# DRSY/EasyKV

Measured on AMD Instinct MI355X. Metric: decode_tokens_per_sec, higher is better.
Workload: dtype f16 storage / f32 accumulate; 1 GPU; bench-D decode at fixed budget: B=1 L=32 Hq=32 H=32 D=128 budget=2048 T=2049 kv_policy=roco (Llama2-7B shape, budget=50% of S=4096); parallelism=1 GPU, layers_per_launch=32, layers_per_rank=32, sequences_per_launch=1, n_split=1, fused=True, slot_map=scattered (random permutation: long-run steady state), prewarm_steps=4096, hipgraph=False, overlap_scorer=False, handoff=False

## Files before the change

easykv_amd/_lib.py:

```python
from __future__ import annotations

import ctypes as C
import os

import torch

from ._build import LIB

POLICY_NONE, POLICY_H2O_HEAD, POLICY_ROCO, POLICY_TOVA, POLICY_RANGE = 0, 1, 2, 3, 4
PHASE_SLOT_TAIL_OK = 32
PHASE_SLOT_ROWS = 16
POLICY_CODES = {"full": POLICY_NONE, "h2o_head": POLICY_H2O_HEAD, "roco": POLICY_ROCO, "tova": POLICY_TOVA,
                "recency": POLICY_RANGE, "random": POLICY_RANGE}

DTYPE_F16, DTYPE_BF16 = 0, 1
DTYPE_CODES = {torch.float16: DTYPE_F16, torch.bfloat16: DTYPE_BF16}

MAX_SEQS = 64
DTYPE_F32 = 2
STEP_CALLS = ("step_check", "step_info", "workspace_bytes", "step_attend")


def step_call_name(rows, batch, what):
    if rows is None and not batch:
        return "ekv_" + what + "_typed"
    return "ekv_" + (rows + "_" if rows else "") + ("batch_" if batch else "") + what


EXPORTS = ("ekv_abi_version", "ekv_strerror", "ekv_workspace_bytes", "ekv_step_plan", "ekv_bank_reset", "ekv_state_init",
           "ekv_step_attend", "ekv_gather_ordered", "ekv_scatter_rows", "ekv_compact_inplace", "ekv_step_check", "ekv_step_info",
           "ekv_rows_to_slots", "ekv_rows_to_order", "ekv_kv8_quantize", "ekv_kv8_dequantize", "ekv_kv4_quantize", "ekv_kv4_dequantize",
           "ekv_kv6_quantize", "ekv_kv6_dequantize", "ekv_set_resident_bytes", "ekv_step_resident_rows", "ekv_kv84_quantize", "ekv_kv84_dequantize",
           "ekv_kv164_quantize", "ekv_kv164_dequantize") + tuple(
               step_call_name(rows, batch, what) for rows in (None, "kv8", "kv4", "kv6", "kv84", "kv164") for batch in (False, True) for what in STEP_CALLS)
LONG_CALLS = {what: "ekv_long_" + what for what in STEP_CALLS}
EXPORTS += tuple(LONG_CALLS[what] for what in STEP_CALLS)
LONG_INFO_N = 12
CAP_CALLS = {what: "ekv_cap_" + what for what in STEP_CALLS}
EXPORTS += tuple(CAP_CALLS[what] for what in STEP_CALLS) + ("ekv_softcap_eval",)
SINK_CALLS = {what: "ekv_sink_" + what for what in STEP_CALLS}
EXPORTS += tuple(SINK_CALLS[what] for what in STEP_CALLS)
WIN_CALLS = {what: "ekv_win_" + what for what in STEP_CALLS}
EXPORTS += tuple(WIN_CALLS[what] for what in STEP_CALLS)
POOL_CALLS = {what: "ekv_pool_" + what for what in STEP_CALLS}
EXPORTS += tuple(POOL_CALLS[what] for what in STEP_CALLS)
POOL_OPS = {"max": 0, "avg": 1}

# ... 72 lines not shown
    lib.ekv_workspace_bytes.restype = C.c_size_t
    lib.ekv_workspace_bytes.argtypes = [C.POINTER(Bank), C.POINTER(Step)]
    lib.ekv_step_plan.argtypes = [C.POINTER(Bank), C.POINTER(Step), C.POINTER(C.c_int32), C.POINTER(C.c_int32)]
    lib.ekv_bank_reset.argtypes = [C.POINTER(Bank), vp]
    lib.ekv_state_init.argtypes = [C.POINTER(Bank), i32, i32, i32, i32, i32, vp]
    lib.ekv_step_attend.argtypes = [C.POINTER(Bank), C.POINTER(Step), vp, vp, vp, vp, vp, vp, vp, vp, C.c_size_t, vp]
    lib.ekv_gather_ordered.argtypes = [C.POINTER(Bank), i32, i32, i32, vp, vp, vp]
    lib.ekv_scatter_rows.argtypes = [C.POINTER(Bank), i32, i32, i32, i32, vp, vp, vp]
    lib.ekv_compact_inplace.argtypes = [C.POINTER(Bank), i32, i32, i32, i32, vp, vp]
    lib.ekv_step_check.argtypes = [C.POINTER(Bank), C.POINTER(Step)]
    lib.ekv_step_info.argtypes = [C.POINTER(Bank), C.POINTER(Step), C.POINTER(C.c_int32), C.c_int32]
    lib.ekv_rows_to_slots.argtypes = [C.POINTER(Bank), i32, i32, i32, vp]
    lib.ekv_rows_to_order.argtypes = [C.POINTER(Bank), i32, i32, i32, vp]
    lib.ekv_set_resident_bytes.argtypes = [C.c_int64]
    lib.ekv_step_resident_rows.argtypes = [C.POINTER(Bank), C.POINTER(Step), i32]
    tails = {"step_check": [], "workspace_bytes": [], "step_info": [C.POINTER(C.c_int32), C.c_int32]}
    for rows, desc in ((None, None), ("kv8", Kv8), ("kv4", Kv4), ("kv6", Kv6), ("kv84", Kv84), ("kv164", Kv164)):
        for batch in (False, True):
            head = [C.POINTER(Bank), C.POINTER(Step), i32] + ([C.POINTER(desc)] if desc else []) + ([C.POINTER(Seq), i32] if batch else [])
            tails["step_attend"] = [vp] * (6 if batch else 8) + [C.c_size_t, vp]
            for what in STEP_CALLS:
                getattr(lib, step_call_name(rows, batch, what)).argtypes = head + tails[what]
        if rows is None:
            tails["step_attend"] = [vp] * 8 + [C.c_size_t, vp]
            for what in STEP_CALLS:
                getattr(lib, LONG_CALLS[what]).argtypes = [C.POINTER(Bank), C.POINTER(Step), i32] + tails[what]
                getattr(lib, CAP_CALLS[what]).argtypes = [C.POINTER(Bank), C.POINTER(Step), i32, C.c_float] + tails[what]
                getattr(lib, SINK_CALLS[what]).argtypes = [C.POINTER(Bank), C.POINTER(Step), i32, vp] + tails[what]
                getattr(lib, WIN_CALLS[what]).argtypes = [C.POINTER(Bank), C.POINTER(Step), i32, C.POINTER(Win)] + tails[what]
                getattr(lib, POOL_CALLS[what]).argtypes = [C.POINTER(Bank), C.POINTER(Step), i32, C.POINTER(Pool)] + tails[what]
# ... 25 lines not shown
```

easykv_amd/csrc/ekv_abi.hip:

```cpp
#include "ekv_common.h"
#include "ekv_kernels.h"
#include "ekv_plan.h"

static inline void drop_stale_error() { (void)hipGetLastError(); }
static inline int launch_code(hipError_t e) { return e == hipSuccess ? EKV_OK : EKV_E_LAUNCH; }

static int call_attend(const EkvCall& c, const void* q, const void* k_new, const void* v_new, void* out, int32_t* evict_ids,
                       const float* rope_cos, const float* rope_sin, void* workspace, size_t workspace_bytes, void* stream) {
  EkvResolved r;
  if (int e = resolve_call(c, &r)) return e;
  const ekv_bank* bank = r.bank;
  const ekv_step* st = r.step;
  const EkvSeqTable* tb = r.tb;
  const EkvStepPlan& P = r.plan;
  if (!q || !k_new || !v_new || !out || !workspace || (st->rope_on_read && (!rope_cos || !rope_sin))) return EKV_E_ARG;
  if (P.bytes > workspace_bytes) return EKV_E_WORKSPACE;
  hipStream_t s = static_cast<hipStream_t>(stream);
  const int n = st->q_len, D = bank->head_dim, lc = st->layer_count;
  char* const ws = static_cast<char*>(workspace);
  auto f32 = [&](int64_t off) { return off < 0 ? nullptr : reinterpret_cast<float*>(ws + off); };
  auto f16 = [&](int64_t off) { return off < 0 ? nullptr : reinterpret_cast<__half*>(ws + off); };

  EkvAttnArgs aa{};
  aa.k = static_cast<const __half*>(bank->k);
// ... 65 lines not shown
  const float* const sinks = P.sink ? c.sinks : nullptr;
  const bool window = P.window != 0;
  const EkvWinArgs win = window ? EkvWinArgs{c.win->tok_pos, c.win->windows, c.win->q_pos0} : EkvWinArgs{};
  drop_stale_error();
  for (int i = 0; i < P.n_list; ++i) {
    const EkvLaunch& L = P.list[i];
    sa.skip_fold = L.skip_fold;
    hipError_t e = hipSuccess;
    if (window && (L.kind == EKV_RUN_CHUNK_LDS || L.kind == EKV_RUN_RESIDENT || L.kind == EKV_RUN_FLUSH || (L.kind == EKV_RUN_CHUNK && P.wide))) return EKV_E_UNSUPPORTED;
    if (rows != EKV_ROWS_kv16 && (L.kind == EKV_RUN_CHUNK_LDS || L.kind == EKV_RUN_RESIDENT || L.kind == EKV_RUN_CHUNK || L.kind == EKV_RUN_FLUSH)) return EKV_E_UNSUPPORTED;
    if (sinks && (L.kind == EKV_RUN_CHUNK_LDS || L.kind == EKV_RUN_RESIDENT || L.kind == EKV_RUN_FLUSH || (L.kind == EKV_RUN_CHUNK && P.wide))) return EKV_E_UNSUPPORTED;
    if (capped && (L.kind == EKV_RUN_CHUNK_LDS || L.kind == EKV_RUN_RESIDENT || L.kind == EKV_RUN_FLUSH || (L.kind == EKV_RUN_CHUNK && P.wide))) return EKV_E_UNSUPPORTED;
    switch (L.kind) {
      case EKV_RUN_FUSED_DECODE:
        aa.fused_order = P.fused_order;
        e = window ? ekv_launch_decode_fused_win(aa, sa, sinks, win, D, lc, P.fused_nw, s, bf16)
          : sinks ? ekv_launch_decode_fused_sink(aa, sa, sinks, D, lc, P.fused_nw, s, bf16)
                  : ekv_launch_decode_fused(aa, sa, tb, D, lc, P.fused_nw, s, bf16, rows, capped);
        break;
      case EKV_RUN_CHUNK_LDS: e = ekv_launch_chunk_lds(aa, sa, D, lc, s, bf16); break;
      case EKV_RUN_RESIDENT: e = ekv_launch_attn_resident(aa, sa, lc, s, bf16); break;
      case EKV_RUN_DECODE:
        e = window ? ekv_launch_attn_decode_win(aa, sinks, win, D, lc, s, bf16)
          : sinks ? ekv_launch_attn_decode_sink(aa, sinks, D, lc, s, bf16) : ekv_launch_attn_decode(aa, tb, D, lc, s, bf16, rows, capped);
        break;
      case EKV_RUN_CHUNK:
        e = window ? ekv_launch_attn_chunk_win(aa, sinks, win, D, lc, P.two_pass, s, L.fuse ? &sa : nullptr, bf16)
          : sinks ? ekv_launch_attn_chunk_sink(aa, sinks, D, lc, P.two_pass, s, L.fuse ? &sa : nullptr, bf16)
                  : ekv_launch_attn_chunk(aa, D, lc, P.wide, P.two_pass, s, L.fuse ? &sa : nullptr, L.passes, L.tail ? &sa : nullptr, bf16, capped);
        break;
// ... 37 lines not shown

int ekv_step_plan(const ekv_bank* bank, const ekv_step* st, int32_t* n_split, int32_t* fused) { return call_plan(bank, st, n_split, fused); }

int ekv_step_info_typed(const ekv_bank* bank, const ekv_step* st, int32_t dtype, int32_t* info, int32_t n_info) {
  return call_info(step_call(bank, st, dtype), info, n_info);
}
int ekv_step_info(const ekv_bank* bank, const ekv_step* st, int32_t* info, int32_t n_info) {
  return call_info(step_call(bank, st, EKV_DTYPE_F16), info, n_info);
}

int ekv_set_resident_bytes(int64_t bytes) {
  ekv_resident_set_budget_bytes(bytes);
  return EKV_OK;
}
int ekv_step_resident_rows(const ekv_bank* bank, const ekv_step* st, int32_t dtype) { return call_resident_rows(step_call(bank, st, dtype)); }

int ekv_step_check_typed(const ekv_bank* bank, const ekv_step* st, int32_t dtype) { return call_check(step_call(bank, st, dtype)); }
int ekv_step_check(const ekv_bank* bank, const ekv_step* st) { return call_check(step_call(bank, st, EKV_DTYPE_F16)); }

int ekv_step_attend(const ekv_bank* bank, const ekv_step* st, const void* q, const void* k_new, const void* v_new,
                    void* out, int32_t* evict_ids, const float* rope_cos, const float* rope_sin, void* workspace,
                    size_t workspace_bytes, void* stream) {
  return call_attend(step_call(bank, st, EKV_DTYPE_F16), q, k_new, v_new, out, evict_ids, rope_cos, rope_sin, workspace, workspace_bytes, stream);
}
int ekv_step_attend_typed(const ekv_bank* bank, const ekv_step* st, int32_t dtype, const void* q, const void* k_new,
                          const void* v_new, void* out, int32_t* evict_ids, const float* rope_cos, const float* rope_sin,
                          void* workspace, size_t workspace_bytes, void* stream) {
  return call_attend(step_call(bank, st, dtype), q, k_new, v_new, out, evict_ids, rope_cos, rope_sin, workspace, workspace_bytes, stream);
}

// ... 398 lines not shown
```

easykv_amd/csrc/ekv_attn_decode.inc:

```
#ifdef EKV_TAIL_PROFILE
#define EKV_STAMP(i) do { if (threadIdx.x == 0) stamps[i] = __builtin_readcyclecounter(); } while (0)
#endif
#include "ekv_decode_stream.h"
#include "ekv_decode_tail.h"
#ifndef EKV_KV8
#define EKV_KV8 0
#endif
#ifndef EKV_BATCH
#define EKV_BATCH 0
#endif
#ifndef EKV_KV4
#define EKV_KV4 0
#endif
#ifndef EKV_KV6
#define EKV_KV6 0
#endif
#if EKV_KV4 || EKV_KV6
#define EKV_MX 1
#else
#define EKV_MX 0
#endif
#ifndef EKV_KV84
#define EKV_KV84 0
#endif
// ... 125 lines not shown
  const int lane = tid & 63, wave = tid >> 6;
  const int T = a.n_slots;
  const int nrep = (REP == 1 || REP == 2) ? REP : a.n_q_heads / a.n_kv_heads;
  const bool roco = sc.policy == EKV_POLICY_ROCO;
  const bool scored = roco || sc.policy == EKV_POLICY_H2O_HEAD || sc.policy == EKV_POLICY_TOVA;
  const int off = scored ? sc.score_off : 0;
  const int W = SLOT ? a.phys_extent : T - off;
  const int w_pad = (int)ekv_align((size_t)W, 256);
#ifdef EKV_NO_PHYS
  constexpr bool PHYS = false;
#else
  constexpr bool PHYS = !ROPE;
#endif
  const int l_pad = a.l_pad;
  constexpr bool kResident = D == 128 && REP == 1 && PHYS && SLOT && !EKV_G8 && !EKV_MX && !EKV_KV164 && !EKV_BATCH && !EKV_SINK && !EKV_WINDOW;
  const int res_rows = kResident ? EKV_RESIDENT_ROWS(a.fused_order) : 0;
  float* s_logit = reinterpret_cast<float*>(smem);
  float* s_part = s_logit + (size_t)REP * l_pad;
  float* sS = s_part + (size_t)Gm::NP * REP * Gm::PS + ((Gm::NP * REP * Gm::PS) & 3 ? 4 - ((Gm::NP * REP * Gm::PS) & 3) : 0);
  float* sQ = sS + w_pad;
  float* sC = sQ + w_pad;
  RedN<NW> red;
  red.buf = reinterpret_cast<unsigned long long*>(sS + (size_t)(roco ? (SLOT ? 2 : 3) : 1) * w_pad);
  red.phase = 0;
  red.lane = lane;
  red.wave = wave;
  const size_t head_row = ((size_t)(a.layer_begin + ll) * a.n_kv_heads + h) * a.cap;
#ifdef EKV_TAIL_PROFILE
  unsigned long long* stamps = reinterpret_cast<unsigned long long*>(sc.tova_row) + ((size_t)ll * a.n_kv_heads + h) * 8;
#endif
  EKV_STAMP(0);
  constexpr bool kOrders = D == 128 && REP == 1 && !ROPE && ((NW == 4 && ITEMS <= 12) || (NW == 8 && !EKV_SOFTCAP && (ITEMS <= 5 || ITEMS == 13))) && SLOT && !EKV_G8 && !EKV_MX && !EKV_KV164 && !EKV_BATCH && !EKV_SINK && !EKV_WINDOW;
  bool order_k = false;
  if constexpr (kOrders) {
    const int om = a.fused_order & 3;
    if (om == 2) {
      order_k = scored;
    } else if (om == 1 && scored) {
      uint32_t* s_flag = reinterpret_cast<uint32_t*>(red.buf);
      if (tid == 0) {
        const uint32_t hw = __builtin_amdgcn_s_getreg(63492);
        const int src = (a.fused_order >> 4) & 3;
        const uint32_t x = src == 0 ? (hw >> 16) & 15u : (src == 1 ? hw & 15u : (uint32_t)(ll * a.n_kv_heads + h));
        bool below = (x & ((a.fused_order >> 8) & 15u)) < ((a.fused_order >> 12) & 15u);
        if constexpr (NW == 8)
          if (src == 3) below = x < (uint32_t)EKV_ORDER_ROUND_THRESHOLD(a.fused_order);
        *s_flag = below != (((a.fused_order >> 6) & 1) != 0) ? 1u : 0u;
      }
      __syncthreads();
      order_k = __builtin_amdgcn_readfirstlane((int)*s_flag) != 0;
    }
  }
// ... 45 lines not shown
      float mk = EKV_NEG_INF;
      ekv_decode_plane_loop<D, NW, kResident>(a.k, head_row, E, mask_ready, [&](uint4 (&kr)[8], const int j0) {
        const unsigned dead8 = (unsigned)s_dead[j0 >> 3];
        float s[8];
#pragma unroll
        for (int u = 0; u < 8; ++u) {
          const float acc = ekv_group_sum<LPR>(ekv_dot8(qv, kr[u], 0.f));
          s[u] = !((dead8 >> u) & 1u) ? EKV_LOGIT(acc, a) : EKV_NEG_INF;
        }
        float mine = s[0];
#pragma unroll
        for (int u = 1; u < 8; ++u) mine = (sub == u) ? s[u] : mine;
        if (sub < 8 && !((dead8 >> sub) & 1u)) s_logit[j0 + sub] = mine;
#pragma unroll
        for (int u = 0; u < 8; ++u) mk = fmaxf(mk, s[u]);
      }, res_rows);
      const __half* v_new_row = a.v_new + ((size_t)ll * a.n_kv_heads + h) * D;
      if (wave == 0 && grp == 0) {
        const uint4 kn = reinterpret_cast<const uint4*>(a.k_new + ((size_t)ll * a.n_kv_heads + h) * D)[sub];
        const uint4 vn = reinterpret_cast<const uint4*>(v_new_row)[sub];
        const size_t off_new = (head_row + new_row) * D;
        reinterpret_cast<uint4*>(a.k_w + off_new)[sub] = kn;
        reinterpret_cast<uint4*>(a.v_w + off_new)[sub] = vn;
        const float acc = EKV_LOGIT(ekv_group_sum<LPR>(ekv_dot8(qv, kn, 0.f)), a);
        if (sub == 0) s_logit[new_row] = acc;
        mk = fmaxf(mk, acc);
      }
      ekv_tail_prefetch_ragged<NW>(sc, head_row, W, roco, sS, sQ, sC, false);
      if constexpr (kLateHeadState) EKV_HEAD_STATE();
      float cC[ITEMS];
      int32_t cB[ITEMS];
// ... 37 lines not shown
#pragma unroll
        for (int u = 1; u < 8; ++u) mx = fmaxf(mx, s[u]);
        const float mn = fmaxf(m[0], mx);
        if (mn == EKV_NEG_INF) return;
        const float alpha = exp2f((m[0] - mn) * EKV_LOG2E);
        l[0] *= alpha;
#pragma unroll
        for (int i = 0; i < 8; ++i) o[0][i] *= alpha;
#pragma unroll
        for (int u = 0; u < 8; ++u) {
          const float p = exp2f((s[u] - mn) * EKV_LOG2E);
          l[0] += p;
          ekv_axpy8(p, vr[u], o[0]);
        }
        m[0] = mn;
      }, res_rows);
      if (wave == 0 && grp == 0) {
        const uint4 vn = reinterpret_cast<const uint4*>(v_new_row)[sub];
        const float acc = s_logit[new_row];
        const float mn = fmaxf(m[0], acc);
        const float alpha = m[0] == EKV_NEG_INF ? 0.f : exp2f((m[0] - mn) * EKV_LOG2E);
        const float p = exp2f((acc - mn) * EKV_LOG2E);
        l[0] = l[0] * alpha + p;
#pragma unroll
        for (int i = 0; i < 8; ++i) o[0][i] *= alpha;
        ekv_axpy8(p, vn, o[0]);
        m[0] = mn;
      }
      ekv_decode_wave_combine<D, 1>(m, l, o);
      ekv_decode_stash<D, 1, NW>(s_part, m, l, o);
      __syncthreads();
// ... 213 lines not shown
```

easykv_amd/csrc/ekv_decode_stream.h:

```cpp
#pragma once
#include "ekv_common.h"
#include "ekv_kernels.h"


struct EkvNoop {
  __device__ __forceinline__ void operator()() const {}
};
#ifndef EKV_ROPE_MOCK
#define EKV_ROPE_MOCK 0
#endif
template <bool RESIDENT>
__device__ __forceinline__ uint4 ekv_load_row_piece(const char* row, int sub) {
  const ekv_u4* p = reinterpret_cast<const ekv_u4*>(row) + sub;
  if constexpr (RESIDENT) return __builtin_bit_cast(uint4, *p);
  else return __builtin_bit_cast(uint4, __builtin_nontemporal_load(p));
}
template <bool B>
struct EkvBool {
  static constexpr bool value = B;
};

template <int D, int REP, bool ROPE, bool SLOT_LDS, int NW = 4, bool PHYS = false, int KU = kU, typename MaskReady = EkvNoop, int EPL = 8, int FMT = 0, bool RES = false>
__device__ __forceinline__ void ekv_decode_stream(const EkvAttnArgs& a, const int32_t* s_slot, float* logit_out,
                                                  int logit_stride, int t0, int t1_in, int ll, int h, size_t head_row,
// ... 546 lines not shown
  ls = 0.f;
  os = 0.f;
#pragma unroll
  for (int i = 0; i < Gm::NP; ++i) {
    const float* p = s_part + ((size_t)i * REP + r) * Gm::PS;
    const float w = (p[0] == EKV_NEG_INF) ? 0.f : exp2f((p[0] - mm) * EKV_LOG2E);
    ls += p[1] * w;
    os += p[2 + d] * w;
  }
}

template <int D, int NW, bool RES = false, typename First, typename Consume>
__device__ __forceinline__ void ekv_decode_plane_loop(const __half* plane, size_t head_row, int t1, First&& first, Consume&& consume, int res_rows = 0) {
  using Gm = EkvDecodeGeom<D, NW, 8, 8>;
  static_assert(Gm::LIVE == Gm::LPR, "whole lane groups");
  constexpr int RW = Gm::RW, STEP = NW * RW;
  const int lane = threadIdx.x & 63, wave = threadIdx.x >> 6;
  const int sub = lane % Gm::LPR, grp = lane / Gm::LPR;
  auto request_as = [&](auto resident, uint4 (&r)[8], int base) {
    int j0 = base + grp * 8;
    if constexpr (RES) asm volatile("" : "+v"(j0));
#pragma unroll
    for (int u = 0; u < 8; ++u) {
      const int row = j0 + u < t1 ? j0 + u : t1 - 1;
      const char* p = reinterpret_cast<const char*>(plane) + (head_row + row) * (D * 2);
      r[u] = ekv_load_row_piece<decltype(resident)::value>(p, sub);
    }
  };
  auto request = [&](uint4 (&r)[8], int base) {
    if constexpr (RES) {
      if (min(base, t1 - 1) < res_rows) request_as(EkvBool<true>(), r, base);
      else request_as(EkvBool<false>(), r, base);
    } else {
      request_as(EkvBool<false>(), r, base);
    }
  };
  uint4 ra[8], rb[8];
  int base = wave * RW;
  request(ra, base);
  first();
  while (base < t1) {
    request(rb, base + STEP);
    consume(ra, base + grp * 8);
    base += STEP;
    if (base >= t1) break;
    request(ra, base + STEP);
// ... 5 lines not shown
```

easykv_amd/csrc/ekv_kernels.h:

```cpp
#pragma once
#include <hip/hip_runtime.h>
#include <hip/hip_fp16.h>
#include <stdint.h>

#include "../../include/easykv_hip.h"
#include "ekv_geometry.h"

enum EkvRows : int32_t { EKV_ROWS_kv16, EKV_ROWS_kv8, EKV_ROWS_kv4, EKV_ROWS_kv6, EKV_ROWS_kv84, EKV_ROWS_kv164 };

#define EKV_RESIDENT_UNIT 32
#define EKV_RESIDENT_BITS(rows) ((((rows) / EKV_RESIDENT_UNIT) > 255 ? 255 : ((rows) / EKV_RESIDENT_UNIT)) << 16)
#define EKV_RESIDENT_ROWS(order) ((((order) >> 16) & 255) * EKV_RESIDENT_UNIT)
#define EKV_ORDER_ROUND_UNIT 8
#define EKV_ORDER_ROUND_BITS(wgs) \
  (((((wgs) / EKV_ORDER_ROUND_UNIT > 255 ? 255 : (wgs) / EKV_ORDER_ROUND_UNIT) >> 4) << 8) | ((((wgs) / EKV_ORDER_ROUND_UNIT > 255 ? 255 : (wgs) / EKV_ORDER_ROUND_UNIT) & 15) << 12))
#define EKV_ORDER_ROUND_THRESHOLD(order) ((((((order) >> 8) & 15) << 4) | (((order) >> 12) & 15)) * EKV_ORDER_ROUND_UNIT)

enum EkvLaunchKind : int32_t {
  EKV_RUN_FUSED_DECODE,
  EKV_RUN_CHUNK_LDS,
  EKV_RUN_RESIDENT,
  EKV_RUN_DECODE,
  EKV_RUN_CHUNK,
  EKV_RUN_FLUSH,
  EKV_RUN_FOLD, EKV_RUN_RANGE, EKV_RUN_DECODE_SCORE, EKV_RUN_TOVA_MEAN, EKV_RUN_SCORE_SELECT,
  EKV_RUN_LONG_FOLD,
  EKV_RUN_LONG_SCORE
// ... 29 lines not shown
  int64_t big_rows;
  int64_t stats, colsum, row_stats;
  int64_t q_keep;
  int64_t q_rot;
  size_t bytes;
  int32_t one_launch;
  int32_t n_launches;
  int32_t n_list;
  EkvLaunch list[6];
  int32_t long_rows, long_tiles;
  int64_t key_rows;
  int32_t capped;
  int32_t sink;
  int32_t window;
  int32_t pooled;
};
struct EkvSeqTable {
  ekv_seq e[EKV_MAX_SEQS];
};

struct EkvAttnArgs {
  const __half* k;
  const __half* v;
  __half* k_w;
  __half* v_w;
  const int32_t* slot_of_pos;
  const __half* q;
  const __half* k_new;
  const __half* v_new;
  float* logits;
// ... 17 lines not shown
  int32_t n_col_parts;
  int32_t n_q_heads, n_kv_heads, cap, n_slots, q_len, n_split, rows_per_split, t_pad, layer_begin, causal;
  int32_t qb_rows, n_qblocks;
  int32_t phys_extent;
  int32_t l_pad;
  uint32_t* arrive;
  float sm_div;
  float softcap;
  __half* q_keep;
  int32_t new_in_cache;
  union {
    int32_t score_tail;
    int32_t fused_order;
  };
  int32_t q_ts, q_hs, kv_ts, kv_hs, o_ts, o_hs;
  int32_t n_stat_parts;
};

struct EkvScoreArgs {
  int32_t* slot_of_pos;
  float* score_sum;
  float* score_sq;
  float* score_cnt;
  const float* logits;
  const float* partials;
  const float* colsum;
  float* big_rows;
  int big_stride;
  const float* row_stats;
  int32_t n_col_parts;
  float* tova_row;
// ... 213 lines not shown
```

easykv_amd/csrc/ekv_plan.cpp:

```cpp
#include "ekv_plan.h"

#include <algorithm>
#include <cstdio>
#include <cstdlib>

namespace {

typedef int64_t i64;

bool env_is_1(const char* name) { const char* e = std::getenv(name); return e != nullptr && e[0] == '1'; }
int env_int(const char* name, int otherwise) { const char* e = std::getenv(name); return e != nullptr ? std::atoi(e) : otherwise; }

bool pow2_to_16(int rep) { return rep == 1 || rep == 2 || rep == 4 || rep == 8 || rep == 16; }

}

int check_bank(const ekv_bank* b) {
  if (!b || !b->k || !b->v || !b->slot_of_pos) return EKV_E_ARG;
  if (b->n_layers <= 0 || b->n_kv_heads <= 0 || b->n_q_heads % b->n_kv_heads || b->cap <= 0) return EKV_E_ARG;
  if (b->head_dim != 32 && b->head_dim != 64 && b->head_dim != 96 && b->head_dim != 128 && b->head_dim != 256) return EKV_E_UNSUPPORTED;
  return EKV_OK;
}

int check_layers(const ekv_bank* b, int begin, int count) {
// ... 56 lines not shown
  return n_heads_in_launch >= 512 ? (1 | rule4) : 0;
}

#ifndef EKV_RESIDENT_MB_DEFAULT
#define EKV_RESIDENT_MB_DEFAULT 224
#endif
namespace {
i64 g_resident_bytes = -1;
}
i64 ekv_resident_budget_bytes() {
  static const i64 dflt = (i64)std::max(0, std::min(env_int("EKV_RESIDENT_MB", EKV_RESIDENT_MB_DEFAULT), 1 << 20)) << 20;
  return g_resident_bytes < 0 ? dflt : g_resident_bytes;
}
void ekv_resident_set_budget_bytes(i64 bytes) { g_resident_bytes = bytes; }

int ekv_decode_resident_rows(i64 n_heads_in_launch, i64 row_bytes, int phys_extent, int cap, int score_rows, i64 budget_bytes) {
  static const int force = env_int("EKV_RESIDENT_ROWS", -1);
  if (n_heads_in_launch <= 0 || row_bytes <= 0 || phys_extent <= 0 || cap <= 0 || score_rows < 0) return 0;
  const i64 unit = EKV_RESIDENT_UNIT;
  const i64 ext = std::min<i64>(((i64)phys_extent + unit - 1) / unit * unit, 255 * unit);
  if (budget_bytes <= 0) return 0;
  if (force >= 0) return (int)std::min<i64>(force / unit * unit, ext);
  const i64 heads = std::min<i64>(n_heads_in_launch, 1 << 20);
  const i64 score = heads * 4 * cap * (score_rows + 2);
  const i64 per_unit = heads * 2 * unit * std::min<i64>(row_bytes, 1 << 16);
  if (budget_bytes < score) return 0;
  return (int)(std::min<i64>((budget_bytes - score) / per_unit, ext / unit) * unit);
}

bool ekv_decode_fused_supported(int head_dim, int rep, int n_slots, int t_pad, int l_pad, int n_evict, int cap, int nw) {
  if (!ekv_attn_decode_supported(head_dim, rep) || rep > 8 || n_evict > 1 || n_slots > 256 * 24 || (cap & 3) != 0 || cap < 16) return false;
  size_t lds = 1 << 30;
  switch (head_dim) {
    case 32: lds = ekv_fused_lds_max<32>(rep, t_pad, l_pad, nw); break;
    case 64: lds = ekv_fused_lds_max<64>(rep, t_pad, l_pad, nw); break;
    case 96: lds = ekv_fused_lds_max<96>(rep, t_pad, l_pad, nw); break;
    case 128: lds = ekv_fused_lds_max<128>(rep, t_pad, l_pad, nw); break;
    case 256: lds = ekv_fused_lds_max<256>(rep, t_pad, l_pad, nw); break;
  }
  return lds <= (size_t)(nw == 8 ? 150 : 80) * 1024;
}

// ... 257 lines not shown
bool plan_whole_step(const StepShape& s, EkvStepPlan* P, int* rc) {
  const ekv_bank* bank = s.bank;
  const ekv_step* st = &s.st;
  const i64 heads_now = (i64)st->layer_count * bank->n_kv_heads;
  *rc = EKV_OK;
  if (s.n == 1 && st->phases == 0 && P->n_split == 1 && !s.pooled &&
      ekv_decode_fused_supported(s.D, s.rep, s.T, P->t_pad, P->l_pad, st->n_evict, bank->cap, P->fused_nw)) {
    if (s.slot_rows && !ekv_slot_rows_supported(bank, st, P->phys_extent, P->t_pad)) {
      *rc = EKV_E_UNSUPPORTED;
      return true;
    }
    P->slot_rows = s.slot_rows ? 1 : 0;
    P->slot_tail_ok = s.slot_rows && s.slot_tail_ok ? 1 : 0;
    P->one_launch = 1;
    P->fused_order = ekv_decode_fused_order(s.D, s.rep, s.scored, s.slot_rows, P->fused_nw, heads_now, P->phys_extent);
    if (s.D == 128 && s.rep == 1 && s.slot_rows && !st->rope_on_read)
      P->fused_order |= EKV_RESIDENT_BITS(ekv_decode_resident_rows(heads_now, 2 * s.D, P->phys_extent, bank->cap,
                                                                   st->policy == EKV_POLICY_ROCO ? 3 : 1, ekv_resident_budget_bytes()));
    run(P, EKV_RUN_FUSED_DECODE, 1);
    return true;
  }
  if (s.slot_rows) {
    *rc = EKV_E_UNSUPPORTED;
    return true;
  }
  if (s.n > 1 && !s.capped && !s.pooled && ekv_chunk_lds_supported(bank, st, P->phys_extent, s.scored) && (heads_now >= 256 || s.T <= 1024)) {
    P->one_launch = 1;
    run(P, EKV_RUN_CHUNK_LDS, 1);
    return true;
  }
  return false;
}

// ... 228 lines not shown
  if (c.sink && c.sinks == nullptr) return EKV_E_ARG;
  if (c.window && !ekv_win_ok(c.win, bank)) return EKV_E_ARG;
  if (c.pooled && !(c.pool != nullptr && c.pool->radius >= 1 && (c.pool->op == EKV_POOL_MAX || c.pool->op == EKV_POOL_AVG))) return EKV_E_ARG;
  const int variants = (c.long_rows ? 1 : 0) + (c.capped ? 1 : 0) + (c.sink || c.window ? 1 : 0) + (c.pooled ? 1 : 0);
  const bool sinkish = c.sink || c.window;
  const int rc = (variants && (quant || c.batch || variants > 1))
                     ? EKV_E_UNSUPPORTED
                     : ekv_plan_step(bank, r->step, P, c.long_rows, c.capped || sinkish, quant || c.batch || sinkish || c.capped, c.pooled);
  P->capped = c.capped ? 1 : 0;
  P->sink = c.sink ? 1 : 0;
  P->window = c.window ? 1 : 0;
  P->pooled = c.pooled ? 1 : 0;
  P->bf16 = c.dtype == EKV_DTYPE_BF16;
  P->rows = c.rows;
  P->batch = c.batch;
  if (quant || c.batch || sinkish) P->fused_order = 0;
  if (c.capped && P->fused_nw == 8) P->fused_order &= ~0xFFFF;
  auto refuse = [&](int code) {
    if (P->long_rows) {
      EkvStepPlan plain;
      (void)ekv_plan_step(bank, r->step, &plain);
      P->bytes = plain.bytes, P->big_rows = plain.big_rows, P->key_rows = -1;
    }
    P->one_launch = P->n_launches = P->n_list = P->long_rows = P->long_tiles = 0;
    if (c.batch || c.capped || sinkish || c.pooled) P->bytes = 0;
    return code;
  };
  const ekv_step* st = c.step;
  if (c.batch) {
    if (int e = check_bank(bank)) return refuse(e);
    if (st->q_len != 1 || st->rope_on_read || st->phases != 0 || st->defer_layers != 0 || st->tova_head_mean) return refuse(EKV_E_UNSUPPORTED);
// ... 59 lines not shown
    if (n_info > 11) info[11] = ok ? P.long_tiles : 0;
  }
  return EKV_OK;
}

int call_resident_rows(const EkvCall& c) {
  EkvResolved r;
  const bool ok = resolve_call(c, &r) == EKV_OK;
  if (c.dtype != EKV_DTYPE_F16 && c.dtype != EKV_DTYPE_BF16) return EKV_E_ARG;
  if (c.rows != EKV_ROWS_kv16 && !r.bank) return EKV_E_ARG;
  if (int e = check_bank(r.bank)) return e;
  if (!c.step || (c.batch && !c.seqs)) return EKV_E_ARG;
  return ok && r.plan.one_launch ? EKV_RESIDENT_ROWS(r.plan.fused_order) : 0;
}

int call_plan(const ekv_bank* bank, const ekv_step* st, int32_t* n_split, int32_t* fused) {
  if (int e = check_bank(bank)) return e;
  if (!st || !n_split || !fused) return EKV_E_ARG;
  EkvResolved r;
  const int rc = resolve_call(step_call(bank, st, EKV_DTYPE_F16), &r);
  *n_split = r.plan.n_split;
  *fused = rc == EKV_OK ? r.plan.one_launch : 0;
  return EKV_OK;
}
```

easykv_amd/csrc/ekv_plan.h:

```cpp
#pragma once
#include "ekv_kernels.h"

int check_bank(const ekv_bank* b);
int check_layers(const ekv_bank* b, int begin, int count);

bool ekv_attn_decode_supported(int head_dim, int rep);
int ekv_decode_fused_nw(int64_t n_heads_in_launch, bool rounds_shape = false);
int ekv_decode_fused_order(int head_dim, int rep, bool scored, bool slot_rows, int nw, int64_t n_heads_in_launch, int phys_extent);
int ekv_decode_resident_rows(int64_t n_heads_in_launch, int64_t row_bytes, int phys_extent, int cap, int score_rows, int64_t budget_bytes);
int64_t ekv_resident_budget_bytes();
void ekv_resident_set_budget_bytes(int64_t bytes);
bool ekv_decode_fused_supported(int head_dim, int rep, int n_slots, int t_pad, int l_pad, int n_evict, int cap, int nw);
bool ekv_decode_score_supported(const EkvScoreArgs& sc);
bool ekv_attn_chunk_supported(int head_dim, int rep, int q_len);
bool ekv_chunk_two_pass(int head_dim, int rep, int q_len, int policy, bool scored, bool accumulate, bool rope, int mode);
bool ekv_chunk_wide(int head_dim, int rep, int q_len, bool rope, bool two_pass, bool wants_logits);
bool ekv_wide_tail_supported(int64_t W, int64_t n_wg);
bool ekv_attn_resident_supported(int head_dim, int rep, int q_len, int n_slots, int64_t W);
bool ekv_chunk_lds_supported(const ekv_bank* bank, const ekv_step* st, int phys_extent, bool scored);
int ekv_attn_chunk_launches(bool wide, bool rope, bool two_pass, int passes);

EkvScoreArgs score_args(const ekv_bank* bank, const ekv_step* st, const EkvStepPlan& P);
int ekv_plan_step(const ekv_bank* bank, const ekv_step* step, EkvStepPlan* P, bool long_rows = false, bool capped = false, bool no_orders = false,
                  bool pooled = false);
// ... 78 lines not shown

struct EkvResolved {
  const ekv_bank* bank;
  const ekv_step* step;
  const EkvSeqTable* tb;
  EkvStepPlan plan;
  ekv_bank bank_q;
  ekv_step env;
  EkvSeqTable table;
};
int resolve_call(const EkvCall& c, EkvResolved* r);
int call_check(const EkvCall& c);
size_t call_workspace_bytes(const EkvCall& c);
int call_info(const EkvCall& c, int32_t* info, int32_t n_info);
int call_resident_rows(const EkvCall& c);
int call_plan(const ekv_bank* bank, const ekv_step* st, int32_t* n_split, int32_t* fused);
```

easykv_amd/engine.py:

```python
from __future__ import annotations

import ctypes as C
import math
from dataclasses import dataclass
from typing import Optional

import torch

from . import _lib
from ._lib import Bank, Step, check

DECODE_RECENT_RATIO = 0.3
ROCO_TAIL = 10


@dataclass
class StepPlan:
    policy: str = "roco"
    phase: str = "decode"
    accumulate: bool = True
    evict: bool = False
    score_off: int = 0
    budget: int = 0
    recent: int = 0
# ... 643 lines not shown
        keys = ("n_split", "fused", "two_pass", "wide", "n_qblocks", "qb_rows", "n_col_parts", "fold_in_kernel", "n_launches", "fused_order",
                "long_scorer", "long_tiles")
        return dict(zip(keys, (int(x) for x in info)))

    def resident_rows(self, plan: StepPlan, q_len=1, layer_begin=0, layer_count=None, phases=0) -> int:
        if self._fmt is not None or self.sinks is not None or self.windows is not None:
            return 0
        st = self.make_step(plan, q_len, layer_begin, self.n_layers - layer_begin if layer_count is None else layer_count)
        st.phases = phases
        _lib.set_resident_bytes(self.resident_bytes)
        rows = self.lib.ekv_step_resident_rows(C.byref(self._bank), C.byref(st), self._dt)
        if rows < 0:
            check(rows, "ekv_step_resident_rows")
        return rows

    def join(self):
        cur = torch.cuda.current_stream(self.device)
        for l, ev in enumerate(self._score_done):
            if ev is not None:
                cur.wait_event(ev)
                self._score_done[l] = None
        self._ws_free = [None] * len(self._ws_free)

    def _attend_overlapped(self, st, q, k_new, v_new, out, evict_ids, lc, layer_begin):
        if self._side is None:
            self._side = [torch.cuda.Stream(self.device) for _ in range(4)]
        main = torch.cuda.current_stream(self.device)
        need = self._step_ws_bytes(st)
        if not self._ws_ring or self._ws_ring[0].numel() < need:
            self._ws_ring = [torch.empty(int(need * 1.25) + 4096, dtype=torch.uint8, device=self.device) for _ in range(8)]
# ... 344 lines not shown
```

include/easykv_hip.h:

```cpp
#ifndef EASYKV_HIP_H
#define EASYKV_HIP_H

#include <stddef.h>
#include <stdint.h>

#ifdef __cplusplus
extern "C" {
#endif

#define EKV_ABI_VERSION 8

enum {
  EKV_POLICY_NONE = 0,
  EKV_POLICY_H2O_HEAD = 1,
  EKV_POLICY_ROCO = 2,
  EKV_POLICY_TOVA = 3,
  EKV_POLICY_RANGE = 4
};

enum {
  EKV_OK = 0,
  EKV_E_ARG = -1,
  EKV_E_UNSUPPORTED = -2,
  EKV_E_WORKSPACE = -3,
// ... 44 lines not shown

int ekv_abi_version(void);
const char *ekv_strerror(int code);

size_t ekv_workspace_bytes(const ekv_bank *bank, const ekv_step *step);
size_t ekv_workspace_bytes_typed(const ekv_bank *bank, const ekv_step *step, int32_t dtype);

int ekv_step_plan(const ekv_bank *bank, const ekv_step *step, int32_t *n_split, int32_t *fused);

#define EKV_STEP_INFO_N 10
int ekv_step_info(const ekv_bank *bank, const ekv_step *step, int32_t *info, int32_t n_info);
int ekv_step_info_typed(const ekv_bank *bank, const ekv_step *step, int32_t dtype, int32_t *info, int32_t n_info);

int ekv_set_resident_bytes(int64_t bytes);
int ekv_step_resident_rows(const ekv_bank *bank, const ekv_step *step, int32_t dtype);

int ekv_bank_reset(const ekv_bank *bank, void *stream);

int ekv_state_init(const ekv_bank *bank, int32_t layer_begin, int32_t layer_count, int32_t width, int32_t mode,
                   int32_t stride, void *stream);

int ekv_step_attend(const ekv_bank *bank, const ekv_step *step, const void *q, const void *k_new, const void *v_new,
                    void *out, int32_t *evict_ids, const float *rope_cos, const float *rope_sin, void *workspace,
                    size_t workspace_bytes, void *stream);
int ekv_step_attend_typed(const ekv_bank *bank, const ekv_step *step, int32_t dtype, const void *q, const void *k_new,
                          const void *v_new, void *out, int32_t *evict_ids, const float *rope_cos, const float *rope_sin,
                          void *workspace, size_t workspace_bytes, void *stream);

int ekv_step_check(const ekv_bank *bank, const ekv_step *step);
int ekv_step_check_typed(const ekv_bank *bank, const ekv_step *step, int32_t dtype);
// ... 221 lines not shown
```

Before: 5993 tokens/s.

## Split resident-row cache budget between K and V planes and use buffer loads

Separates the resident (cache-retained) row count for the K and V planes, splitting the byte budget by a configurable percentage (default 50/50), so that V reads can stay cache-resident independently of K. Row loads in the decode plane loop switch to raw buffer loads with a bounded resource descriptor, which removes the per-row clamp arithmetic, and the cache policy bit is chosen from residency. A shortcut also lets the order decision for 8-wave scored launches come from a plan bit instead of a runtime flag. Behaviour changes for the over-range rows because the loop no longer clamps to t1-1, and the cache split may cost K residency.

```diff
diff --git a/easykv_amd/_lib.py b/easykv_amd/_lib.py
--- a/easykv_amd/_lib.py
+++ b/easykv_amd/_lib.py
@@ -30,7 +30,7 @@
 EXPORTS = ("ekv_abi_version", "ekv_strerror", "ekv_workspace_bytes", "ekv_step_plan", "ekv_bank_reset", "ekv_state_init",
            "ekv_step_attend", "ekv_gather_ordered", "ekv_scatter_rows", "ekv_compact_inplace", "ekv_step_check", "ekv_step_info",
            "ekv_rows_to_slots", "ekv_rows_to_order", "ekv_kv8_quantize", "ekv_kv8_dequantize", "ekv_kv4_quantize", "ekv_kv4_dequantize",
-           "ekv_kv6_quantize", "ekv_kv6_dequantize", "ekv_set_resident_bytes", "ekv_step_resident_rows", "ekv_kv84_quantize", "ekv_kv84_dequantize",
+           "ekv_kv6_quantize", "ekv_kv6_dequantize", "ekv_set_resident_bytes", "ekv_step_resident_rows", "ekv_step_resident_rows_v", "ekv_kv84_quantize", "ekv_kv84_dequantize",
            "ekv_kv164_quantize", "ekv_kv164_dequantize") + tuple(
                step_call_name(rows, batch, what) for rows in (None, "kv8", "kv4", "kv6", "kv84", "kv164") for batch in (False, True) for what in STEP_CALLS)
 LONG_CALLS = {what: "ekv_long_" + what for what in STEP_CALLS}
@@ -133,6 +133,7 @@
     lib.ekv_rows_to_order.argtypes = [C.POINTER(Bank), i32, i32, i32, vp]
     lib.ekv_set_resident_bytes.argtypes = [C.c_int64]
     lib.ekv_step_resident_rows.argtypes = [C.POINTER(Bank), C.POINTER(Step), i32]
+    lib.ekv_step_resident_rows_v.argtypes = [C.POINTER(Bank), C.POINTER(Step), i32]
     tails = {"step_check": [], "workspace_bytes": [], "step_info": [C.POINTER(C.c_int32), C.c_int32]}
     for rows, desc in ((None, None), ("kv8", Kv8), ("kv4", Kv4), ("kv6", Kv6), ("kv84", Kv84), ("kv164", Kv164)):
         for batch in (False, True):
diff --git a/easykv_amd/csrc/ekv_abi.hip b/easykv_amd/csrc/ekv_abi.hip
--- a/easykv_amd/csrc/ekv_abi.hip
+++ b/easykv_amd/csrc/ekv_abi.hip
@@ -103,6 +103,7 @@
     switch (L.kind) {
       case EKV_RUN_FUSED_DECODE:
         aa.fused_order = P.fused_order;
+        aa.resident_v = P.resident_v;
         e = window ? ekv_launch_decode_fused_win(aa, sa, sinks, win, D, lc, P.fused_nw, s, bf16)
           : sinks ? ekv_launch_decode_fused_sink(aa, sa, sinks, D, lc, P.fused_nw, s, bf16)
                   : ekv_launch_decode_fused(aa, sa, tb, D, lc, P.fused_nw, s, bf16, rows, capped);
@@ -170,6 +171,7 @@
   return EKV_OK;
 }
 int ekv_step_resident_rows(const ekv_bank* bank, const ekv_step* st, int32_t dtype) { return call_resident_rows(step_call(bank, st, dtype)); }
+int ekv_step_resident_rows_v(const ekv_bank* bank, const ekv_step* st, int32_t dtype) { return call_resident_rows_v(step_call(bank, st, dtype)); }
 
 int ekv_step_check_typed(const ekv_bank* bank, const ekv_step* st, int32_t dtype) { return call_check(step_call(bank, st, dtype)); }
 int ekv_step_check(const ekv_bank* bank, const ekv_step* st) { return call_check(step_call(bank, st, EKV_DTYPE_F16)); }
diff --git a/easykv_amd/csrc/ekv_attn_decode.inc b/easykv_amd/csrc/ekv_attn_decode.inc
--- a/easykv_amd/csrc/ekv_attn_decode.inc
+++ b/easykv_amd/csrc/ekv_attn_decode.inc
@@ -163,7 +163,9 @@
 #endif
   const int l_pad = a.l_pad;
   constexpr bool kResident = D == 128 && REP == 1 && PHYS && SLOT && !EKV_G8 && !EKV_MX && !EKV_KV164 && !EKV_BATCH && !EKV_SINK && !EKV_WINDOW;
-  const int res_rows = kResident ? EKV_RESIDENT_ROWS(a.fused_order) : 0;
+  const int res_rows_k = kResident ? EKV_RESIDENT_ROWS(a.fused_order) : 0;
+  const int res_rows_v = kResident ? EKV_RESIDENT_V_ROWS(a.resident_v) : 0;
+  const int res_rows = min(res_rows_k, res_rows_v);
   float* s_logit = reinterpret_cast<float*>(smem);
   float* s_part = s_logit + (size_t)REP * l_pad;
   float* sS = s_part + (size_t)Gm::NP * REP * Gm::PS + ((Gm::NP * REP * Gm::PS) & 3 ? 4 - ((Gm::NP * REP * Gm::PS) & 3) : 0);
@@ -185,6 +187,8 @@
     const int om = a.fused_order & 3;
     if (om == 2) {
       order_k = scored;
+    } else if (NW == 8 && om == 1 && scored && ((a.fused_order >> 4) & 3) == 3 && EKV_ORDER_ROUND_THRESHOLD(a.fused_order) == 0) {
+      order_k = ((a.fused_order >> 6) & 1) != 0;
     } else if (om == 1 && scored) {
       uint32_t* s_flag = reinterpret_cast<uint32_t*>(red.buf);
       if (tid == 0) {
@@ -260,7 +264,7 @@
         if (sub < 8 && !((dead8 >> sub) & 1u)) s_logit[j0 + sub] = mine;
 #pragma unroll
         for (int u = 0; u < 8; ++u) mk = fmaxf(mk, s[u]);
-      }, res_rows);
+      }, res_rows_k);
       const __half* v_new_row = a.v_new + ((size_t)ll * a.n_kv_heads + h) * D;
       if (wave == 0 && grp == 0) {
         const uint4 kn = reinterpret_cast<const uint4*>(a.k_new + ((size_t)ll * a.n_kv_heads + h) * D)[sub];
@@ -328,7 +332,7 @@
           ekv_axpy8(p, vr[u], o[0]);
         }
         m[0] = mn;
-      }, res_rows);
+      }, res_rows_v);
       if (wave == 0 && grp == 0) {
         const uint4 vn = reinterpret_cast<const uint4*>(v_new_row)[sub];
         const float acc = s_logit[new_row];
diff --git a/easykv_amd/csrc/ekv_decode_stream.h b/easykv_amd/csrc/ekv_decode_stream.h
--- a/easykv_amd/csrc/ekv_decode_stream.h
+++ b/easykv_amd/csrc/ekv_decode_stream.h
@@ -584,22 +584,22 @@
 __device__ __forceinline__ void ekv_decode_plane_loop(const __half* plane, size_t head_row, int t1, First&& first, Consume&& consume, int res_rows = 0) {
   using Gm = EkvDecodeGeom<D, NW, 8, 8>;
   static_assert(Gm::LIVE == Gm::LPR, "whole lane groups");
-  constexpr int RW = Gm::RW, STEP = NW * RW;
+  constexpr int RW = Gm::RW, STEP = NW * RW, ROWB = D * 2;
   const int lane = threadIdx.x & 63, wave = threadIdx.x >> 6;
   const int sub = lane % Gm::LPR, grp = lane / Gm::LPR;
+  const __amdgpu_buffer_rsrc_t rows = __builtin_amdgcn_make_buffer_rsrc(
+      const_cast<char*>(reinterpret_cast<const char*>(plane)) + head_row * ROWB, 0, t1 * ROWB, 0x00020000);
   auto request_as = [&](auto resident, uint4 (&r)[8], int base) {
     int j0 = base + grp * 8;
     if constexpr (RES) asm volatile("" : "+v"(j0));
-#pragma unroll
-    for (int u = 0; u < 8; ++u) {
-      const int row = j0 + u < t1 ? j0 + u : t1 - 1;
-      const char* p = reinterpret_cast<const char*>(plane) + (head_row + row) * (D * 2);
-      r[u] = ekv_load_row_piece<decltype(resident)::value>(p, sub);
-    }
+    constexpr int kPolicy = decltype(resident)::value ? 0 : 2;
+    const int off = j0 * ROWB + sub * 16;
+#pragma unroll
+    for (int u = 0; u < 8; ++u) r[u] = __builtin_bit_cast(uint4, __builtin_amdgcn_raw_buffer_load_b128(rows, off + u * ROWB, 0, kPolicy));
   };
   auto request = [&](uint4 (&r)[8], int base) {
     if constexpr (RES) {
-      if (min(base, t1 - 1) < res_rows) request_as(EkvBool<true>(), r, base);
+      if (base < res_rows) request_as(EkvBool<true>(), r, base);
       else request_as(EkvBool<false>(), r, base);
     } else {
       request_as(EkvBool<false>(), r, base);
diff --git a/easykv_amd/csrc/ekv_kernels.h b/easykv_amd/csrc/ekv_kernels.h
--- a/easykv_amd/csrc/ekv_kernels.h
+++ b/easykv_amd/csrc/ekv_kernels.h
@@ -11,6 +11,8 @@
 #define EKV_RESIDENT_UNIT 32
 #define EKV_RESIDENT_BITS(rows) ((((rows) / EKV_RESIDENT_UNIT) > 255 ? 255 : ((rows) / EKV_RESIDENT_UNIT)) << 16)
 #define EKV_RESIDENT_ROWS(order) ((((order) >> 16) & 255) * EKV_RESIDENT_UNIT)
+#define EKV_RESIDENT_V_BITS(rows) (((rows) / EKV_RESIDENT_UNIT) > 255 ? 255 : ((rows) / EKV_RESIDENT_UNIT))
+#define EKV_RESIDENT_V_ROWS(word) (((word) & 255) * EKV_RESIDENT_UNIT)
 #define EKV_ORDER_ROUND_UNIT 8
 #define EKV_ORDER_ROUND_BITS(wgs) \
   (((((wgs) / EKV_ORDER_ROUND_UNIT > 255 ? 255 : (wgs) / EKV_ORDER_ROUND_UNIT) >> 4) << 8) | ((((wgs) / EKV_ORDER_ROUND_UNIT > 255 ? 255 : (wgs) / EKV_ORDER_ROUND_UNIT) & 15) << 12))
@@ -70,6 +72,7 @@
   int32_t sink;
   int32_t window;
   int32_t pooled;
+  int32_t resident_v;
 };
 struct EkvSeqTable {
   ekv_seq e[EKV_MAX_SEQS];
@@ -117,7 +120,10 @@
     int32_t fused_order;
   };
   int32_t q_ts, q_hs, kv_ts, kv_hs, o_ts, o_hs;
-  int32_t n_stat_parts;
+  union {
+    int32_t n_stat_parts;
+    int32_t resident_v;
+  };
 };
 
 struct EkvScoreArgs {
diff --git a/easykv_amd/csrc/ekv_plan.cpp b/easykv_amd/csrc/ekv_plan.cpp
--- a/easykv_amd/csrc/ekv_plan.cpp
+++ b/easykv_amd/csrc/ekv_plan.cpp
@@ -94,18 +94,36 @@
 }
 void ekv_resident_set_budget_bytes(i64 bytes) { g_resident_bytes = bytes; }
 
-int ekv_decode_resident_rows(i64 n_heads_in_launch, i64 row_bytes, int phys_extent, int cap, int score_rows, i64 budget_bytes) {
+#ifndef EKV_RESIDENT_SPLIT_DEFAULT
+#define EKV_RESIDENT_SPLIT_DEFAULT 50
+#endif
+int ekv_resident_split_percent() {
+  static const int pct = std::max(0, std::min(env_int("EKV_RESIDENT_SPLIT", EKV_RESIDENT_SPLIT_DEFAULT), 100));
+  return pct;
+}
+
+int ekv_decode_resident_rows(i64 n_heads_in_launch, i64 row_bytes, int phys_extent, int cap, int score_rows, i64 budget_bytes, int split_percent,
+                             int* rows_v) {
   static const int force = env_int("EKV_RESIDENT_ROWS", -1);
+  static const int force_v = env_int("EKV_RESIDENT_ROWS_V", -1);
+  int none = 0;
+  int& rv = rows_v ? *rows_v : none;
+  rv = 0;
   if (n_heads_in_launch <= 0 || row_bytes <= 0 || phys_extent <= 0 || cap <= 0 || score_rows < 0) return 0;
   const i64 unit = EKV_RESIDENT_UNIT;
   const i64 ext = std::min<i64>(((i64)phys_extent + unit - 1) / unit * unit, 255 * unit);
   if (budget_bytes <= 0) return 0;
-  if (force >= 0) return (int)std::min<i64>(force / unit * unit, ext);
   const i64 heads = std::min<i64>(n_heads_in_launch, 1 << 20);
   const i64 score = heads * 4 * cap * (score_rows + 2);
-  const i64 per_unit = heads * 2 * unit * std::min<i64>(row_bytes, 1 << 16);
-  if (budget_bytes < score) return 0;
-  return (int)(std::min<i64>((budget_bytes - score) / per_unit, ext / unit) * unit);
+  const i64 per_plane = heads * unit * std::min<i64>(row_bytes, 1 << 16);
+  const i64 kv = budget_bytes < score ? -1 : std::min<i64>(budget_bytes - score, (i64)1 << 50);
+  const i64 pct = std::max(0, std::min(split_percent, 100));
+  i64 rk = kv < 0 ? 0 : std::min<i64>(kv * pct / (100 * per_plane), ext / unit) * unit;
+  i64 rvv = kv < 0 ? 0 : std::min<i64>(kv * (100 - pct) / (100 * per_plane), ext / unit) * unit;
+  if (force >= 0) rk = rvv = std::min<i64>(force / unit * unit, ext);
+  if (force_v >= 0) rvv = std::min<i64>(force_v / unit * unit, ext);
+  rv = (int)rvv;
+  return (int)rk;
 }
 
 bool ekv_decode_fused_supported(int head_dim, int rep, int n_slots, int t_pad, int l_pad, int n_evict, int cap, int nw) {
@@ -393,9 +411,12 @@
     P->slot_tail_ok = s.slot_rows && s.slot_tail_ok ? 1 : 0;
     P->one_launch = 1;
     P->fused_order = ekv_decode_fused_order(s.D, s.rep, s.scored, s.slot_rows, P->fused_nw, heads_now, P->phys_extent);
-    if (s.D == 128 && s.rep == 1 && s.slot_rows && !st->rope_on_read)
-      P->fused_order |= EKV_RESIDENT_BITS(ekv_decode_resident_rows(heads_now, 2 * s.D, P->phys_extent, bank->cap,
-                                                                   st->policy == EKV_POLICY_ROCO ? 3 : 1, ekv_resident_budget_bytes()));
+    if (s.D == 128 && s.rep == 1 && s.slot_rows && !st->rope_on_read) {
+      int rows_v = 0;
+      P->fused_order |= EKV_RESIDENT_BITS(ekv_decode_resident_rows(heads_now, 2 * s.D, P->phys_extent, bank->cap, st->policy == EKV_POLICY_ROCO ? 3 : 1,
+                                                                   ekv_resident_budget_bytes(), ekv_resident_split_percent(), &rows_v));
+      P->resident_v = EKV_RESIDENT_V_BITS(rows_v);
+    }
     run(P, EKV_RUN_FUSED_DECODE, 1);
     return true;
   }
@@ -654,7 +675,7 @@
   P->bf16 = c.dtype == EKV_DTYPE_BF16;
   P->rows = c.rows;
   P->batch = c.batch;
-  if (quant || c.batch || sinkish) P->fused_order = 0;
+  if (quant || c.batch || sinkish) P->fused_order = P->resident_v = 0;
   if (c.capped && P->fused_nw == 8) P->fused_order &= ~0xFFFF;
   auto refuse = [&](int code) {
     if (P->long_rows) {
@@ -744,6 +765,13 @@
   return ok && r.plan.one_launch ? EKV_RESIDENT_ROWS(r.plan.fused_order) : 0;
 }
 
+int call_resident_rows_v(const EkvCall& c) {
+  EkvResolved r;
+  const bool ok = resolve_call(c, &r) == EKV_OK;
+  const int rows_k = call_resident_rows(c);
+  return rows_k < 0 ? rows_k : (ok && r.plan.one_launch ? EKV_RESIDENT_V_ROWS(r.plan.resident_v) : 0);
+}
+
 int call_plan(const ekv_bank* bank, const ekv_step* st, int32_t* n_split, int32_t* fused) {
   if (int e = check_bank(bank)) return e;
   if (!st || !n_split || !fused) return EKV_E_ARG;
diff --git a/easykv_amd/csrc/ekv_plan.h b/easykv_amd/csrc/ekv_plan.h
--- a/easykv_amd/csrc/ekv_plan.h
+++ b/easykv_amd/csrc/ekv_plan.h
@@ -7,7 +7,9 @@
 bool ekv_attn_decode_supported(int head_dim, int rep);
 int ekv_decode_fused_nw(int64_t n_heads_in_launch, bool rounds_shape = false);
 int ekv_decode_fused_order(int head_dim, int rep, bool scored, bool slot_rows, int nw, int64_t n_heads_in_launch, int phys_extent);
-int ekv_decode_resident_rows(int64_t n_heads_in_launch, int64_t row_bytes, int phys_extent, int cap, int score_rows, int64_t budget_bytes);
+int ekv_decode_resident_rows(int64_t n_heads_in_launch, int64_t row_bytes, int phys_extent, int cap, int score_rows, int64_t budget_bytes,
+                             int split_percent = 50, int* rows_v = nullptr);
+int ekv_resident_split_percent();
 int64_t ekv_resident_budget_bytes();
 void ekv_resident_set_budget_bytes(int64_t bytes);
 bool ekv_decode_fused_supported(int head_dim, int rep, int n_slots, int t_pad, int l_pad, int n_evict, int cap, int nw);
@@ -116,4 +118,5 @@
 size_t call_workspace_bytes(const EkvCall& c);
 int call_info(const EkvCall& c, int32_t* info, int32_t n_info);
 int call_resident_rows(const EkvCall& c);
+int call_resident_rows_v(const EkvCall& c);
 int call_plan(const ekv_bank* bank, const ekv_step* st, int32_t* n_split, int32_t* fused);
diff --git a/easykv_amd/engine.py b/easykv_amd/engine.py
--- a/easykv_amd/engine.py
+++ b/easykv_amd/engine.py
@@ -681,6 +681,17 @@
             check(rows, "ekv_step_resident_rows")
         return rows
 
+    def resident_rows_v(self, plan: StepPlan, q_len=1, layer_begin=0, layer_count=None, phases=0) -> int:
+        if self._fmt is not None or self.sinks is not None or self.windows is not None:
+            return 0
+        st = self.make_step(plan, q_len, layer_begin, self.n_layers - layer_begin if layer_count is None else layer_count)
+        st.phases = phases
+        _lib.set_resident_bytes(self.resident_bytes)
+        rows = self.lib.ekv_step_resident_rows_v(C.byref(self._bank), C.byref(st), self._dt)
+        if rows < 0:
+            check(rows, "ekv_step_resident_rows_v")
+        return rows
+
     def join(self):
         cur = torch.cuda.current_stream(self.device)
         for l, ev in enumerate(self._score_done):
diff --git a/include/easykv_hip.h b/include/easykv_hip.h
--- a/include/easykv_hip.h
+++ b/include/easykv_hip.h
@@ -82,6 +82,7 @@
 
 int ekv_set_resident_bytes(int64_t bytes);
 int ekv_step_resident_rows(const ekv_bank *bank, const ekv_step *step, int32_t dtype);
+int ekv_step_resident_rows_v(const ekv_bank *bank, const ekv_step *step, int32_t dtype);
 
 int ekv_bank_reset(const ekv_bank *bank, void *stream);
 
```

Result: no change. 5992 tokens/s, median of 2 (-0.0%).
